# NeLy-EPFL/flygym

Hardware: AMD Instinct MI355X
Metric: env-steps/sec (whole node), 4096 flies per GPU, flat terrain (higher is better)
Workload: dtype f32

## Files before the change

flygym_amd/_native.py:

```python

from __future__ import annotations

import ctypes
import os
import subprocess
from pathlib import Path

PKG = Path(__file__).resolve().parent
LIB_PATH = Path(os.environ["NMF_HIP_LIB"]) if os.environ.get("NMF_HIP_LIB") else PKG / "libnmf_hip.so"
MATH_FLAGS = ["-fno-hip-fp32-correctly-rounded-divide-sqrt", "-freciprocal-math", "-fno-signed-zeros", "-fassociative-math", "-fno-trapping-math", "-fno-math-errno", "-fapprox-func"]
CSRC = PKG / "csrc"
INCLUDE = PKG.parent / "include"

FIELDS = dict(
    qpos=0, qvel=1, ctrl=2, qacc_warmstart=3, seg_xpos=4, seg_xquat=5, site_xpos=6,
    actuator_force=7, sensordata=8, time=9, stats=10, qacc=11, cost=12, stats_sum=13, contact_geom=14, act=15,
)

INT_FIELDS = frozenset({"stats_sum"})

_lib = None


class NativeError(RuntimeError):
    pass


class BatchOptions(ctypes.Structure):

    _fields_ = [("struct_size", ctypes.c_int32), ("solver", ctypes.c_int32), ("sched", ctypes.c_int32), ("order", ctypes.c_int32),
                ("max_chunks", ctypes.c_int32), ("min_chunk_steps", ctypes.c_int32), ("order_every", ctypes.c_int32),
                ("rest_slow", ctypes.c_int32), ("chunk_div", ctypes.c_float), ("flies_per_cu", ctypes.c_int32)]

    SOLVER = {"": 0, "default": 0, "primal": 1, "nohist": 2, "nofallback": 4}
    SCHED = {"": 0, "chunks": 0, "plain": 1}
    ORDER = {"": 0, "auto": 0, "inorder": 1, "costliest": 2, "none": 3, "policy": 4}

    @classmethod
    def make(cls, solver="", sched="", order="", max_chunks=0, min_chunk_steps=0, order_every=0, rest_slow=False, chunk_div=0.0,
             flies_per_cu=0):
        return cls(ctypes.sizeof(cls), cls.SOLVER[solver], cls.SCHED[sched], cls.ORDER[order], int(max_chunks), int(min_chunk_steps),
                   int(order_every), int(bool(rest_slow)), float(chunk_div), int(flies_per_cu))


INFO_KEYS = ("kernel_family", "terrain_kernel", "tether_kernel", "contact_space_flavour", "contact_space_max_contacts", "flies_per_cu",
             "resident_workgroups", "chunked", "max_chunks", "chunk_div_x1000", "order_policy", "solver_option_bits", "noslip_iterations",
             "contact_capacity", "kernel_lds_bytes", "kernel_vgprs")


def build(force: bool = False, verbose: bool = False) -> Path:
    srcs = [CSRC / "nmf_capi.hip", CSRC / "nmf_step.hip", CSRC / "nmf_sensors.hip", CSRC / "nmf_eyes.hip", CSRC / "nmf_replay.hip", CSRC / "nmf_device.h", CSRC / "nmf_tree.h", CSRC / "nmf_dual.h",
            INCLUDE / "nmf.h", Path(__file__)]
    if os.environ.get("NMF_HIP_LIB"):
        return LIB_PATH
    def fresh():
        return LIB_PATH.exists() and all(LIB_PATH.stat().st_mtime >= s.stat().st_mtime for s in srcs)

    if not force and fresh():
        return LIB_PATH
    import fcntl

    lock = open(LIB_PATH.with_suffix(".lock"), "w")
    fcntl.flock(lock, fcntl.LOCK_EX)
    try:
        if not force and fresh():
            return LIB_PATH
        return _compile(verbose)
    finally:
        fcntl.flock(lock, fcntl.LOCK_UN)
        lock.close()


def _compile(verbose: bool) -> Path:
    tmp = LIB_PATH.with_name(LIB_PATH.name + f".{os.getpid()}.tmp")
    cmd = [
        "hipcc", "--offload-arch=gfx950", "-O3", "-std=c++17", "-fno-slp-vectorize", "-mllvm", "-amdgpu-sched-strategy=iterative-ilp",
        *MATH_FLAGS, "-mllvm", "-amdgpu-atomic-optimizer-strategy=None", "-fPIC", "-shared",
        f"-I{INCLUDE}", f"-I{CSRC}", str(CSRC / "nmf_capi.hip"), "-o", str(tmp),
    ]
    res = subprocess.run(cmd, capture_output=True, text=True)
    if res.returncode != 0:
        tmp.unlink(missing_ok=True)
        raise NativeError("hipcc failed:\n" + res.stderr[-4000:])
    if verbose:
        print(res.stderr)
    os.replace(tmp, LIB_PATH)
    return LIB_PATH
# ... 71 lines not shown
```

flygym_amd/csrc/nmf_capi.hip:

```cpp
#include <hip/hip_runtime.h>

#include <algorithm>
#include <cmath>
#include <cstdio>
#include <cstdlib>
#include <cstring>
#include <string>
#include <vector>

#include "nmf.h"
#include "nmf_step.hip"
#include "nmf_sensors.hip"
#include "nmf_eyes.hip"
#include "nmf_replay.hip"

namespace {

thread_local std::string g_err;
int fail(const std::string& msg) { g_err = msg; return -1; }

#define HIP_OK(expr)                                                                        \
  do {                                                                                      \
    hipError_t e_ = (expr);                                                                 \
    if (e_ != hipSuccess) return fail(std::string(#expr) + ": " + hipGetErrorString(e_));   \
// ... 268 lines not shown
  int n_chunks = 1;
  b->st.n_chunks = 1; b->st.csched = b->csched_buf; b->st.handoff = b->handoff_buf; b->st.handoff_stride = b->handoff_stride;
  if (oversub && b->chunking && b->csched_buf && b->handoff_buf && n_steps >= 2 * b->min_chunk_steps) {
    int start = 0, c = 0;
    while (start < n_steps && c < b->max_chunks) {
      const double div = !b->chunk_div_short ? b->chunk_div : n_steps > 64 ? 2.0 : (b->chunk_div < 1.75 && n_steps <= 30 ? 1.6 : b->chunk_div);
      int len = (int)std::ceil((n_steps - start) / div);
      len = std::max(len, b->min_chunk_steps);
      if (c == b->max_chunks - 1 || n_steps - start - len < b->min_chunk_steps) len = n_steps - start;
      b->st.chunk_start[c++] = start;
      start += len;
    }
    b->st.chunk_start[c] = n_steps;
    n_chunks = c;
    b->st.n_chunks = c;
  }
  b->st.sched_mode = n_chunks > 1 ? 1 : 0;
  dim3 grid(n_chunks > 1 ? (unsigned)std::min(b->resident_waves, b->n_worlds * n_chunks) : (unsigned)b->n_worlds), block(nmf::kWave);
  b->st.order = nullptr; b->st.sched = nullptr;
  if (oversub && b->order_buf && b->sched_buf && b->order_policy != 2) {
    const int policy = b->order_policy == 3 ? (n_steps <= 64 ? 1 : -1) : b->order_policy;
    if (!(policy == 1 && b->order_valid && ++b->order_age < b->order_every)) {
      hipLaunchKernelGGL(nmf::nmf_order_kernel, dim3(1), dim3(1024), 0, stream, b->st.cost, b->n_worlds, b->order_buf, b->sched_buf, n_steps, policy);
      b->order_age = 0; b->order_valid = true;
    }
    b->st.order = b->order_buf;
    if (policy < 0) b->st.sched = b->sched_buf;
  }
  const nmf::DevModel* dm = b->dm_dev;
  nmf::ReplayArgs rp_arg = rp;
  void* args[] = {&dm, &b->st, &rp_arg, &n_steps};
  (void)hipLaunchKernel(b->step_fn, grid, block, args, b->lds_pad, stream);
  HIP_OK(hipGetLastError());
  return 0;
}

const char* dev_env(const char* name) {
  static const bool allowed = [] { const char* e = getenv("NMF_ALLOW_ENV"); return e && atoi(e) != 0; }();
  return allowed ? getenv(name) : nullptr;
}

struct Options {
  int solver = 0, sched = 0, order = 0, max_chunks = 0, min_chunk_steps = 0, order_every = 0, rest_slow = 0, flies_per_cu = 0;
  double chunk_div = 0.0;
};

Options read_options(const nmf_batch_options& in) {
  Options o;
  o.solver = in.solver; o.sched = in.sched; o.order = in.order; o.max_chunks = in.max_chunks; o.min_chunk_steps = in.min_chunk_steps;
  o.order_every = in.order_every; o.rest_slow = in.rest_slow; o.flies_per_cu = in.flies_per_cu;
  if (in.chunk_div > 1.f) o.chunk_div = in.chunk_div;
  if (const char* e = dev_env("NMF_SOLVER")) {
    const std::string v(e);
    o.solver = v == "primal" ? 1 : v == "nohist" ? 2 : v == "nofallback" ? 4 : 0;
  }
  if (const char* e = dev_env("NMF_SCHED")) o.sched = std::string(e) == "plain" ? 1 : 0;
  if (const char* e = dev_env("NMF_ORDER")) {
    const std::string v(e);
    o.order = v == "inorder" ? 1 : v == "costliest" ? 2 : v == "none" ? 3 : v == "policy" ? 4 : 0;
  }
  if (const char* e = dev_env("NMF_ORDER_EVERY")) o.order_every = std::max(1, atoi(e));
  if (const char* e = dev_env("NMF_MAX_CHUNKS")) o.max_chunks = std::max(1, std::min(16, atoi(e)));
  if (const char* e = dev_env("NMF_CHUNK_DIV")) o.chunk_div = std::max(1.0, atof(e));
  if (const char* e = dev_env("NMF_MIN_CHUNK_STEPS")) o.min_chunk_steps = std::max(1, atoi(e));
  if (const char* e = dev_env("NMF_FLIES_PER_CU")) o.flies_per_cu = atoi(e);
  if (dev_env("NMF_DISABLE_REST_FAST")) o.rest_slow = 1;
  return o;
}

struct Skeleton {
  int topo = -1;
  std::vector<int> tree_body, child_start, child_count, lvl_start;
};

int classify_skeleton(const nmf_model* model, Skeleton& sk) {
  int& topo = sk.topo;
  if (model->star[0] == 1 && model->star[1] == 6 && model->star[2] == 11 && model->star[3] == 8) topo = 0;
  if (model->star[0] == 1 && model->star[1] == 6 && model->star[2] == 7 && model->star[3] == 4) topo = 1;
  if (topo >= 0) {
    const HostArray* dn = model->find("body_dofnum");
    const int pat0[8] = {3, 2, 1, 1, 1, 1, 1, 1}, pat1[4] = {3, 2, 1, 1};
    const int* pat = topo == 0 ? pat0 : pat1;
    const int nbl = topo == 0 ? 8 : 4;
    bool ok = dn && dn->is_int && (int)dn->i.size() == 1 + 6 * nbl && dn->i[0] == 6;
    for (int b = 1; ok && b < 1 + 6 * nbl; ++b) ok = dn->i[(size_t)b] == pat[(b - 1) % nbl];
    if (!ok || model->nu > nmf::kMaxCtrl) topo = -1;
  }
  std::vector<char> in_tree;
  if (topo < 0) {
    const HostArray* bp = model->find("body_parent");
    const HostArray* dn = model->find("body_dofnum");
    const int patB[8] = {3, 2, 1, 1, 1, 1, 1, 1}, patA[8] = {3, 3, 3, 3, 3, 3, 3, 3};
    for (int cand = 4; cand <= 5 && topo < 0 && bp && dn; ++cand) {
      const int* pat = cand == 4 ? patB : patA;
      const int nb = model->nb, lb0 = 21, want_nv = cand == 4 ? 132 : 210;
      bool ok = nb == 69 && model->nv == want_nv && (int)dn->i.size() == nb && dn->i[0] == 6 && model->nu <= (cand == 4 ? nmf::FlyTopoBio::kCtrl : nmf::FlyTopoAll::kCtrl);
      int rest_v = 0;
      for (int bb = 1; ok && bb < lb0; ++bb) { rest_v += dn->i[(size_t)bb]; ok = bp->i[(size_t)bb] >= 0 && bp->i[(size_t)bb] < lb0 && bp->i[(size_t)bb] < bb; }
      ok = ok && rest_v == 60;
      for (int bb = lb0; ok && bb < nb; ++bb) {
        const int l = (bb - lb0) % 8;
        ok = dn->i[(size_t)bb] == pat[l] && bp->i[(size_t)bb] == (l == 0 ? 0 : bb - 1);
      }
      if (ok) { topo = cand; in_tree.assign((size_t)nb, 0); for (int bb = 0; bb < lb0; ++bb) in_tree[(size_t)bb] = 1; }
    }
  }
  std::vector<int> &tree_body = sk.tree_body, &child_start = sk.child_start, &child_count = sk.child_count, &lvl_start = sk.lvl_start;
// ... 67 lines not shown
  UI(body_dofadr); UI(body_dofnum); UI(dof_body);
  UF(dof_axis); UF(dof_armature); UF(dof_damping); UF(dof_stiffness); UF(dof_springref);
  UI(seg_body); UF(seg_pos); UF(seg_quat); UI(site_body); UF(site_pos);
  UI(act_type); UI(act_trn); UI(act_limited); UI(act_geom); UF(act_gain); UF(act_bias); UF(act_forcerange); UF(act_ctrlrange);
  UF(key_qpos); UF(key_ctrl);
  d.act_general = nullptr;
  if (const HostArray* ag = model->find("act_general")) {
    if (ag->is_int || (int)ag->f.size() != model->nu * nmf::kActGen) { rc |= fail("nmf_batch_create: act_general must be float [nu][32]"); }
    else {
      UF(act_general);
      std::vector<int> trn = model->find("act_trn")->i;
      for (int u = 0; u < model->nu; ++u) if ((int)ag->f[(size_t)u * nmf::kActGen] & 1) trn[(size_t)u] = 0;
      rc |= upload(b, trn, reinterpret_cast<const int**>((void*)&d.act_trn));
    }
  }
  UI(geom_body); UI(geom_type); UI(geom_hulladr); UI(geom_hullnum); UI(geom_sensor);
  UF(geom_p0); UF(geom_p1); UF(geom_radius); UF(geom_bsphere); UF(geom_invweight0); UF(hull_vert);
  UF(pair_friction); UF(pair_solref); UF(pair_solimp); UF(pair_margin);
#undef UF
#undef UI
  if (topo >= 2) {
    const HostArray* bp = model->find("body_parent");
    rc |= upload(b, bp->i, reinterpret_cast<const int**>((void*)&d.body_parent));
    rc |= upload(b, tree_body, reinterpret_cast<const int**>((void*)&d.tree_body));
    rc |= upload(b, child_start, reinterpret_cast<const int**>((void*)&d.tree_child_start));
    rc |= upload(b, child_count, reinterpret_cast<const int**>((void*)&d.tree_child_count));
    d.tree_nlevel = (int)lvl_start.size() - 1;
    for (size_t k = 0; k < 18; ++k) d.tree_lvl_start[k] = k < lvl_start.size() ? lvl_start[k] : (int)tree_body.size();
    d.rest_fast = 0; d.rest_pack = nullptr;
    if (topo >= 4) {
      const HostArray* dn = model->find("body_dofnum");
      const HostArray* da = model->find("body_dofadr");
      const int nl = (int)lvl_start.size() - 2;
      bool fast = da && nl <= nmf::kRestLevels && !opt.rest_slow;
      std::vector<int> pack((size_t)nmf::kRestLevels * 16, -1);
      for (int lv = 1; fast && lv <= nl; ++lv) {
        const int k0 = lvl_start[(size_t)lv], k1 = lvl_start[(size_t)lv + 1];
        fast = k1 - k0 <= 8;
        for (int k = k0; fast && k < k1; ++k) {
          const int bb = tree_body[(size_t)k];
          fast = dn->i[(size_t)bb] == 3 && da->i[(size_t)bb] < 256 && child_count[(size_t)bb] < 256 && child_start[(size_t)bb] < 256;
          pack[(size_t)((lv - 1) * 8 + (k - k0)) * 2] = bb | (bp->i[(size_t)bb] << 8) | (da->i[(size_t)bb] << 16) | (child_count[(size_t)bb] << 24);
          pack[(size_t)((lv - 1) * 8 + (k - k0)) * 2 + 1] = child_start[(size_t)bb] | (k << 8);
        }
      }
      if (fast) { d.rest_fast = 1; const int* pp = nullptr; rc |= upload(b, pack, &pp); *reinterpret_cast<const int**>((void*)&d.rest_pack) = pp; }
    }
  } else {
    d.body_parent = d.tree_body = d.tree_child_start = d.tree_child_count = nullptr; d.tree_nlevel = 0; d.rest_fast = 0; d.rest_pack = nullptr;
  }
  d.noslip_iter = 0;
  if (const HostArray* os2 = model->find("opt_solver")) { if (os2->i.size() > 1) d.noslip_iter = os2->i[1]; }
  d.max_contacts = nmf::kMaxCon;
  d.solver_flags = opt.solver & 7;
  if (rc != 0) return rc;
  void* p = nullptr;
  if (hipMalloc(&p, sizeof(nmf::DevModel)) != hipSuccess) return fail("nmf_batch_create: model upload failed");
  b->allocs.push_back(p); b->dm_dev = (nmf::DevModel*)p;
  if (hipMemcpy(p, &d, sizeof(nmf::DevModel), hipMemcpyHostToDevice) != hipSuccess) return fail("nmf_batch_create: model upload failed");
  return 0;
}

int alloc_state(nmf_batch* b) {
  const nmf_model* model = b->model;
  const size_t n_worlds = (size_t)b->n_worlds;
  nmf::DevState& st = b->st;
  st.n_worlds = b->n_worlds;
  float* stats_sum = nullptr;
  b->handoff_stride = (model->nq + 2 * model->nv + model->nu + 6 + nmf::kActHistWords + 63) / 64 * 64;
  if (alloc_field(b, NMF_QPOS, model->nq, &st.qpos) || alloc_field(b, NMF_QVEL, model->nv, &st.qvel) ||
      alloc_field(b, NMF_CTRL, model->nu, &st.ctrl) || alloc_field(b, NMF_QACC_WARMSTART, model->nv, &st.qacc_ws) ||
      alloc_field(b, NMF_SEG_XPOS, model->nseg * 3, &st.seg_xpos) || alloc_field(b, NMF_SEG_XQUAT, model->nseg * 4, &st.seg_xquat) ||
      alloc_field(b, NMF_SITE_XPOS, model->nsite * 3, &st.site_xpos) || alloc_field(b, NMF_ACTUATOR_FORCE, model->nu, &st.actuator_force) ||
      alloc_field(b, NMF_SENSORDATA, 96, &st.sensordata) || alloc_field(b, NMF_TIME, 1, &st.time) ||
      alloc_field(b, NMF_STATS, 8, &st.stats) || alloc_field(b, NMF_QACC, model->nv, &st.qacc) || alloc_field(b, NMF_COST, 1, &st.cost) ||
      alloc_field(b, NMF_STATS_SUM, 16, &stats_sum) ||
      alloc_field(b, NMF_CONTACT_GEOM, nmf::kMaxCon, &st.contact_geom) || alloc_field(b, NMF_ACT, model->nu, &st.act) ||
      alloc_dev(b, n_worlds, &b->order_buf, false) || alloc_dev(b, 1, &b->csched_buf) ||
      alloc_dev(b, n_worlds * (size_t)b->handoff_stride, &b->handoff_buf) ||
      alloc_dev(b, n_worlds * nmf::kActHistWords, &st.act_hist))
    return -1;
  st.stats_sum = reinterpret_cast<unsigned int*>(stats_sum);
  st.dual_scratch = nullptr;
  if (b->topo == 5 && alloc_dev(b, n_worlds * nmf::kDualScratchFloats, &st.dual_scratch, false)) return -1;
  st.noslip_buf = nullptr;
  if (b->dm.noslip_iter > 0 && alloc_dev(b, n_worlds * nmf::kNoslipFloats, &st.noslip_buf)) return -1;
  if (alloc_dev(b, 2, &b->clock_probe_buf) || alloc_dev(b, 1, &b->sched_buf)) return -1;
  st.clock_probe = b->clock_probe_buf;
  st.sched = nullptr;
  st.order = nullptr;
  return 0;
}

void set_schedule(nmf_batch* b, const Options& opt) {
  b->chunking = opt.sched != 1;
  if (opt.order) b->order_policy = opt.order == 1 ? 0 : opt.order == 2 ? 1 : opt.order == 3 ? 2 : opt.order == 4 ? -1 : 3;
  if (opt.order_every > 0) b->order_every = opt.order_every;
  if (opt.max_chunks > 0) b->max_chunks = std::max(1, std::min(16, opt.max_chunks));
  b->chunk_div = (b->dm.terrain_type == 0 && b->topo < 2) ? 1.7 : 2.0;
  b->chunk_div_short = true;
  if (opt.chunk_div > 0.0) { b->chunk_div = opt.chunk_div; b->chunk_div_short = false; }
  if (opt.min_chunk_steps > 0) b->min_chunk_steps = opt.min_chunk_steps;
  if (b->dm.act_general) b->chunking = false;
}

int pick_kernel(nmf_batch* b, const Options& opt) {
  const int topo = b->topo, device = b->device;
// ... 564 lines not shown
```

flygym_amd/csrc/nmf_dual.h:

```cpp
#pragma once

namespace nmf {

template <class TP>
__device__ __forceinline__ float* dual_g(FlyLds<TP>& s) {
  constexpr size_t need = sizeof(float) * dual_g_floats(kDualMaxCon<TP>);
  if constexpr (kDualH<TP>) {
    static_assert(!kDualH<TP> || need <= sizeof(s.T) + sizeof(s.W), "G does not fit T..W");
    return &s.T[0][0];
  } else {
    static_assert(kDualH<TP> || need <= sizeof(s.Ib) + sizeof(s.T) + sizeof(s.W) + sizeof(s.dual_pad), "G does not fit Ib..W");
    return &s.Ib[0][0];
  }
}
struct DualCol {
  lds_cptr G;
  int cc;
  int cc9b, blk9b;
  int tdb, td3b;
  float smu;
  float alpha, beta;
  struct Raw { float nn, nt, tn, tt, smu2, a2; };
  __device__ __forceinline__ void init(const float* g, int lane, float smu_) {
    G = lds_pinned(g); cc = lane >> 2; cc9b = 36 * cc; blk9b = 36 * (cc * (cc + 1) / 2);
    const int td = 1 + ((lane >> 1) & 1);
    tdb = 4 * td; td3b = 12 * td; smu = smu_;
    alpha = 1.f; beta = smu_;
    asm("" : "+v"(cc9b), "+v"(blk9b), "+v"(tdb), "+v"(td3b));
  }
  __device__ __forceinline__ Raw fetch(int kk) const {
    const unsigned int c2 = (unsigned int)kk >> 2, td2b = 4u + (((unsigned int)kk << 1) & 4u);
    int c29b = (int)(36u * c2), blk29b = (int)(18u * (c2 * (c2 + 1u)));
    asm("" : "+s"(c29b), "+s"(blk29b));
    int lo = blk9b + c29b, up = cc9b + blk29b;
    asm("" : "+v"(lo), "+v"(up));
    const bool ge = cc >= (int)c2;
    const int base = ge ? lo : up;
    const int o_nt = (ge ? 1 : 3) * (int)td2b, o_tn = ge ? td3b : tdb;
    const int a_nt = base + o_nt, a_tn = base + o_tn, a_tt = a_tn + o_nt;
    auto at = [&](int byte_off) { return *(lds_cptr)((const __attribute__((address_space(3))) char*)G + byte_off); };
    Raw r;
    r.nn = at(base); r.nt = at(a_nt); r.tn = at(a_tn); r.tt = at(a_tt);
    r.smu2 = readlane_f(beta, kk); r.a2 = readlane_f(alpha, kk);
    return r;
  }
  __device__ __forceinline__ float value(const Raw& r) const { return fmaf(beta, fmaf(r.smu2, r.tt, r.a2 * r.tn), alpha * fmaf(r.smu2, r.nt, r.a2 * r.nn)); }
};
__device__ __forceinline__ float quad_sum(float v) {
  v += NMF_DPP(v, 0xB1);
  v += NMF_DPP(v, 0x4E);
  return v;
}
constexpr int dual_root_axis(int i) { return i < 3 ? 2 - i : 8 - i; }

template <int PMAX>
__device__ __forceinline__ void dual_eliminate(unsigned long long rem, const DualCol& dc, float R, int lane, float& b, float& diag) {
  float cq[PMAX];
  auto first_of = [](unsigned long long r) { return __builtin_amdgcn_readfirstlane(max(__ffsll((long long)r) - 1, 0)); };
  int kk_next = first_of(rem);
  DualCol::Raw an = dc.fetch(kk_next);
#define NMF_DUAL_PIVOT(P)                                                                                   \
  if constexpr (P < PMAX) {                                                                                 \
    if (rem == 0ull) return;                                                                                \
    const int kk = kk_next;                                                                                 \
    rem &= rem - 1ull;                                                                                      \
    float col = dc.value(an) + (lane == kk ? R : 0.f);                                                      \
    kk_next = first_of(rem);                                                                                \
    an = dc.fetch(kk_next);                                                                                 \
    __builtin_amdgcn_sched_barrier(0);       \
    { float c1 = 0.f;                                                                                       \
      _Pragma("unroll") for (int q = 0; q + 1 < P; q += 2) {                                                \
        col = fmaf(-cq[q], readlane_f(cq[q], kk), col); c1 = fmaf(-cq[q + 1], readlane_f(cq[q + 1], kk), c1); } \
      if constexpr ((P) % 2) col = fmaf(-cq[P - 1], readlane_f(cq[P - 1], kk), col);                        \
      col += c1; }                                                                                          \
    const float d = readlane_f(col, kk);                                                                    \
    const float rs = __builtin_amdgcn_rsqf(d);                                                              \
    diag = lane == kk ? d : diag;                                                                           \
    const float cp = lane == kk ? 0.f : col * rs;                                                           \
    b = fmaf(-cp, readlane_f(b, kk) * rs, b);                                                               \
    cq[P] = cp;                                                                                             \
  }
#define NMF_DUAL_PIVOT8(P) NMF_DUAL_PIVOT(P) NMF_DUAL_PIVOT(P + 1) NMF_DUAL_PIVOT(P + 2) NMF_DUAL_PIVOT(P + 3) NMF_DUAL_PIVOT(P + 4) NMF_DUAL_PIVOT(P + 5) NMF_DUAL_PIVOT(P + 6) NMF_DUAL_PIVOT(P + 7)
  NMF_DUAL_PIVOT8(0) NMF_DUAL_PIVOT8(8) NMF_DUAL_PIVOT8(16) NMF_DUAL_PIVOT8(24) NMF_DUAL_PIVOT8(32) NMF_DUAL_PIVOT8(40) NMF_DUAL_PIVOT8(48) NMF_DUAL_PIVOT8(56)
#undef NMF_DUAL_PIVOT8
#undef NMF_DUAL_PIVOT
}

template <class TP>
__device__ __noinline__ void dual_restore(FlyLds<TP>& s, const GModel& m, int lane) {
  WSYNC();
  if constexpr (kDualS<TP>) {
    for (int b = lane; b < TP::NB; b += kWave) {
      const float* Q = s.Isym[b];
      float* I = s.Ib[b];
      I[0] = Q[15]; I[1] = Q[13]; I[2] = Q[5]; I[3] = Q[8]; I[4] = Q[0]; I[5] = Q[6]; I[6] = Q[11]; I[7] = Q[1]; I[8] = Q[2]; I[9] = Q[7];
    }
    WSYNC();
  }
  sweep_twists(s, s.qacc_smooth, s.T, m, lane);
}

template <class TP>
__device__ __forceinline__ float dual_noslip(FlyLds<TP>& s, const GModel& m, int lane, int ncon, float frow, float j0, float R, float smu) {
  lane = opaque(lane);
  ncon = __builtin_amdgcn_readfirstlane(ncon);
  const bool on = lane < 4 * ncon;
  const float scale = 1.0f / (m.meaninertia * (float)TP::NV);
  DualCol dcol;
  dcol.init(dual_g(s), lane, smu);
    for (int sweep = 0; sweep < m.noslip_iter; ++sweep) {
      float improvement = sweep == 0 ? wave_sum(0.5f * frow * frow * R) : 0.f;
      for (int c2 = 0; c2 < ncon; ++c2) {
        for (int pp = 0; pp < 2; ++pp) {
          const int r0 = 4 * c2 + 2 * pp, r1 = r0 + 1;
          const float col0 = dcol.value(dcol.fetch(r0)), col1 = dcol.value(dcol.fetch(r1));
          const float res0 = wave_sum(on ? col0 * frow : 0.f) + readlane_f(j0, r0), res1 = wave_sum(on ? col1 * frow : 0.f) + readlane_f(j0, r1);
          const float a00 = readlane_f(col0, r0), a01 = readlane_f(col0, r1), a11 = readlane_f(col1, r1);
          const float old0 = readlane_f(frow, r0), old1 = readlane_f(frow, r1);
          const float bc0 = res0 - a00 * old0 - a01 * old1, bc1 = res1 - a01 * old0 - a11 * old1;
          const float mid = 0.5f * (old0 + old1);
          const float K1 = a00 + a11 - 2.f * a01, K0 = mid * (a00 - a11) + bc0 - bc1;
          float n0 = mid, n1 = mid;
          if (!(K1 < kMinVal)) { const float y = fminf(fmaxf(-K0 / K1, -mid), mid); n0 = mid + y; n1 = mid - y; }
          const float d0 = n0 - old0, d1 = n1 - old1;
          float change = 0.5f * (d0 * (a00 * d0 + a01 * d1) + d1 * (a01 * d0 + a11 * d1)) + d0 * res0 + d1 * res1;
          if (change > 1e-10f) { n0 = old0; n1 = old1; change = 0.f; }
          frow = lane == r0 ? n0 : lane == r1 ? n1 : frow;
          improvement -= change;
        }
      }
      if (scale * improvement < 1e-6f) break;
    }
  return frow;
}
template <class TP>
__device__ __noinline__ float dual_noslip_cold(FlyLds<TP>& s, const GModel& m, int lane, int ncon, float frow, float j0, float R, float smu) {
// ... 123 lines not shown
  SUB(43);
  {
    const int kd = k < 3 ? k : 2;
    const int half = ncon >> 1;
    for (int t = 0; t <= half; ++t) {
      int c2 = cc - t;
      c2 = c2 < 0 ? c2 + ncon : c2;
      const int src = (on ? 4 * c2 + k : lane) << 2;
      auto from = [&](float v) { return __builtin_bit_cast(float, __builtin_amdgcn_ds_bpermute(src, __builtin_bit_cast(int, v))); };
      float pr[6], pl[NDL];
#pragma unroll
      for (int i = 0; i < 6; ++i) pr[i] = from(ur[i]);
#pragma unroll
      for (int d = 0; d < NDL; ++d) pl[d] = from(ul[d]);
      const bool same = __builtin_amdgcn_ds_bpermute(src, leg) == leg;
      const bool ge = cc >= c2;
      int base = ge ? 9 * (cc * (cc + 1) / 2 + c2) + 3 * kd : 9 * (c2 * (c2 + 1) / 2 + cc) + kd;
      const int stride = ge ? 1 : 3;
      asm("" : "+v"(base));
      static_for<3>([&](auto PP) {
        constexpr int p = decltype(PP)::value;
        auto rot = [&](float v) {
          if constexpr (p == 0) return v; else if constexpr (p == 1) return NMF_DPP(v, 0xC9); else return NMF_DPP(v, 0xD2);
        };
        float a = rot(pr[0]) * ur[0];
#pragma unroll
        for (int i = 1; i < 6; ++i) a = fmaf(rot(pr[i]), ur[i], a);
        float bl = rot(pl[0]) * ul[0];
#pragma unroll
        for (int d = 1; d < NDL; ++d) bl = fmaf(rot(pl[d]), ul[d], bl);
        a += same ? bl : 0.f;
        const int d2 = kd + p >= 3 ? kd + p - 3 : kd + p;
        if (on && k < 3) Gm[base + stride * d2] = a;
      });
    }
  }
  WSYNC();
  SUB(44);
  STAGE(9);

  float jar = fmaf(c_ws, je, j0), lam = 0.f;
  DualCol dcol;
  dcol.init(Gm, lane, smu);
  const float scale = 1.0f / (m.meaninertia * (float)TP::NV);
  int iters = 0;
  bool guessed = hist_any && !(m.solver_flags & 2);
  int stalls = 0;
  unsigned int exit_bit = kExitMaxIter;
  int npiv = 0;
  float jar_last = 0.f;
  unsigned long long viol_last = 0ull;
  unsigned long long mask_p = ~0ull, mask_pp = ~0ull;
  unsigned long long mask = guessed ? __ballot(on && (hist_nib ? ((hist_nib >> k) & 1) != 0 : jar < 0.f)) : __ballot(on && jar < 0.f);
  for (int iter = 0; iter < m.max_iter; ++iter) {
    iters = iter + 1;
    const unsigned int nib4 = (unsigned int)(mask >> (4 * cc)) & 0xfu;
#ifdef NMF_DUAL_DIRS
    const bool fullc = on && nib4 == 0xfu && mu > 1e-6f;
#else
    const bool fullc = false;
#endif
    float b, diag = 1.f, R_e = R;
    unsigned long long mask_e = mask;
    {
      const float q0 = NMF_DPP(j0, 0x00), q1 = NMF_DPP(j0, 0x55), q2 = NMF_DPP(j0, 0xAA), q3 = NMF_DPP(j0, 0xFF);
      const float hm = 0.5f * __builtin_amdgcn_rcpf(mu);
      const float bdir = k == 0 ? 0.25f * ((q0 + q1) + (q2 + q3)) : k == 1 ? hm * (q0 - q1) : k == 2 ? hm * (q2 - q3) : 0.f;
      b = fullc ? bdir : j0;
      R_e = fullc ? (k == 0 ? 0.25f * R : R * (2.f * hm * hm)) : R;
      dcol.alpha = fullc ? (k == 0 ? 1.f : 0.f) : 1.f;
      dcol.beta = fullc ? ((k == 1 || k == 2) ? 1.f : 0.f) : smu;
      mask_e = __ballot(fullc ? k < 3 : (bool)((mask >> lane) & 1ull));
    }
    dual_eliminate<4 * NC>(mask_e, dcol, R_e, lane, b, diag);
    const bool act = (mask >> lane) & 1ull;
    const bool piv = (mask_e >> lane) & 1ull;
    const float x = piv ? -b * __builtin_amdgcn_rcpf(diag) : 0.f;
    float lam_t, jar_t;
    {
      const float x0 = NMF_DPP(x, 0x00), x1 = NMF_DPP(x, 0x55), x2 = NMF_DPP(x, 0xAA);
      const float hm = 0.5f * __builtin_amdgcn_rcpf(mu);
      const float lam_dir = fmaf((k & 1) ? -hm : hm, k < 2 ? x1 : x2, 0.25f * x0);
      lam_t = fullc ? lam_dir : (act ? x : 0.f);
      jar_t = fullc ? -R * lam_dir : (act ? -R * lam_t : b);
    }
    dcol.alpha = 1.f; dcol.beta = smu;
    const unsigned long long tmask = __ballot(on && jar_t < 0.f);
    npiv = max(npiv, (int)__popcll(mask_e));
    jar_last = jar_t; viol_last = tmask ^ mask;
#ifdef NMF_DUAL_DEBUG
    {
      const float dmin = wave_min(act ? diag : 1e30f), lmax = wave_max(on ? fabsf(lam_t) : 0.f), jmax = wave_max(on ? fabsf(jar_t) : 0.f);
      const float amax = wave_max(on ? fabsf(dcol.value(dcol.fetch(0))) : 0.f);
      if (blockIdx.x == 0 && lane == 0) printf("iter %d npiv %d mask %016llx tmask %016llx min pivot %g max|lam_t| %g max|jar_t| %g max diag A %g c %g\n", iter, __popcll(mask), mask, tmask, dmin, lmax, jmax, amax, c_ws);
    }
#endif
    STAGE(10);
    if (tmask == mask) {
      lam = lam_t; jar = jar_t; c_ws = 0.f;
      exit_bit = kExitKkt;
      break;
    }
    if (iter >= 2 && mask == mask_pp) {
      const bool off = on && (((tmask ^ mask) >> lane) & 1ull);
      const float viol = wave_max(off ? fabsf(jar_t) : 0.f), all = wave_max(on ? fabsf(jar_t) : 0.f);
      if (viol <= 1e-3f * all) { lam = lam_t; jar = jar_t; c_ws = 0.f; exit_bit = kExitTie; break; }
    }
    mask_pp = mask_p; mask_p = mask;
    const float jv = jar_t - jar, dlam = lam_t - lam, dc = -c_ws;
    float g1, g2, s1, s2;
    {
      const float Alam = jar - j0 - c_ws * je, Adlam = fmaf(c_ws, je, jv);
      const bool neg = on && jar < 0.f;
      const float S1 = wave_sum(on ? je * lam : 0.f), S2 = wave_sum(on ? je * dlam : 0.f);
      const float S3 = wave_sum(on ? dlam * Alam : 0.f), S4 = wave_sum(on ? dlam * Adlam : 0.f);
      s1 = wave_sum(neg ? D * jar * jv : 0.f); s2 = wave_sum(neg ? D * jv * jv : 0.f);
      g1 = c_ws * dc * eMe + dc * S1 + c_ws * S2 + S3;
      g2 = dc * dc * eMe + 2.f * dc * S2 + S4;
    }
    STAGE(11);
    float alpha = 0.f, lo = 0.f, hi = -1.f;
    for (int ls = 0; ls < 30; ++ls) {
      float d1 = s1 + g1, d2 = s2 + g2;
      if (ls > 0) {
        const float x = fmaf(alpha, jv, jar);
        const bool neg = on && x < 0.f;
        d1 = wave_sum(neg ? D * x * jv : 0.f) + g1 + alpha * g2;
// ... 173 lines not shown
```

flygym_amd/csrc/nmf_step.hip:

```cpp
#include "nmf_device.h"

namespace nmf {

#define WSYNC() do { __builtin_amdgcn_fence(__ATOMIC_SEQ_CST, "wavefront"); __builtin_amdgcn_wave_barrier(); } while (0)
#ifndef NMF_TOPO_MASK
#define NMF_TOPO_MASK 0x3f
#endif
#define NMF_HAS_TOPO(k) ((NMF_TOPO_MASK >> (k)) & 1)
constexpr float kNoiseFactor = 8.f;
enum : unsigned int {
  kExitDual = 1u << 8,
  kExitKkt = 1u << 9,
  kExitTie = 1u << 10,
  kExitStall = 1u << 11,
  kExitCost = 1u << 12,
  kExitMaxIter = 1u << 13,
  kExitPrimal = 1u << 14,
  kExitFallback = 1u << 15,
  kExitBigPivots = 1u << 16,
  kExitNoNoslip = 1u << 17,
  kExitFree = 1u << 18,
};
constexpr int kExitKinds = 12;
constexpr int kDualRegPivots = 47;
// ... 59 lines not shown
  float fact[TP::kNFact][8];
  float slot[TP::kNSlot][27];
  int rt_nb, rt_nv;
  NMF_TREE_TABLES
};
template <class TP>
struct TreeLds<TP, true, true> {
  float fact[TP::kNFact][8];
  int reduced;
  float restA[21];
  unsigned int t_pack[kRestLevels][8][2];
  NMF_TREE_TABLES
};

template <class TP> constexpr bool has_cm3() { if constexpr (TP::kStar) return TP::REST_B == 0; else return false; }
template <class TP> inline constexpr bool kHasCm3 = has_cm3<TP>();
template <class TP> inline constexpr bool kHasIsym = has_cm3<TP>();

constexpr bool rows_conflict_free(int rows_per_leg, int width, int nleg) {
  const int ng = nleg < 4 ? nleg : 4;
  for (int a = 0; a < ng; ++a)
    for (int b = a + 1; b < ng; ++b) {
      const int d = (((b - a) * rows_per_leg * width) % 32 + 32) % 32;
      if (d < 6 || d > 26) return false;
    }
  return true;
}
constexpr int conflict_free_width(int rows_per_leg, int nleg) {
  for (int w = 6; w <= 9; ++w) if (rows_conflict_free(rows_per_leg, w, nleg)) return w;
  return 6;
}
template <class TP> constexpr int row_width_s() { if constexpr (TP::kStar) return TP::REST_B == 0 ? conflict_free_width(TP::NDL, TP::NLEG) : 6; else return 6; }
template <class TP> constexpr int row_width_tw() { if constexpr (TP::kStar) return TP::REST_B == 0 ? conflict_free_width(TP::NBL, TP::NLEG) : 6; else return 6; }
template <class TP> constexpr bool dual_hybrid() {
  if constexpr (TP::kStar) return TP::REST_B > 0; else return false;
}
template <class TP> constexpr bool dual_global() {
  if constexpr (TP::kStar) return TP::REST_B > 0 && 4 * TP::NV < TP::NLEG * TP::NDL * 8; else return false;
}
template <class TP> inline constexpr bool kDualS = has_cm3<TP>();
template <class TP> inline constexpr bool kDualH = dual_hybrid<TP>();
template <class TP> inline constexpr bool kDual = kDualS<TP> || kDualH<TP>;
template <class TP> inline constexpr bool kDualGlob = kDualH<TP> && dual_global<TP>();
constexpr int kDualScratchFloats = 8 * 6 * 24;
constexpr int dual_g_floats(int ncon) { return 9 * ncon * (ncon + 1) / 2; }
template <class TP> constexpr int dual_max_con() {
  if constexpr (kDualH<TP>) {
    int n = 0;
    while (n < 16 && dual_g_floats(n + 1) <= 2 * TP::NB * 6) ++n;
    return n;
  } else return 16;
}
template <class TP> inline constexpr int kDualMaxCon = dual_max_con<TP>();
template <class TP> inline constexpr int kHistLds = kDualS<TP> ? kActHistWords : kDualH<TP> ? 5 : 0;
template <class TP, class M> __device__ __forceinline__ int hist_words(const M& m) {
  if constexpr (kDualS<TP>) return (m.ng + 1) / 2; else return kHistLds<TP>;
}
template <class TP> constexpr int dual_pad_floats() {
  if constexpr (kDualS<TP>) {
    constexpr int need = dual_g_floats(kDualMaxCon<TP>);
    constexpr int have = TP::NB * 11 + 2 * TP::NB * (TP::REST_B == 0 ? conflict_free_width(TP::NBL, TP::NLEG) : 6);
    return need > have ? need - have : 0;
  } else return 0;
}

struct HotModel {
  const float *dof_axis, *body_pos, *body_quat, *geom_p0, *geom_p1, *geom_radius, *geom_bsphere, *hull_vert, *pair_margin;
  const int *geom_body, *geom_type, *geom_hulladr, *geom_hullnum;
  float plane[4], terrain[5], hull_skin;
  int terrain_type, ng, sem_max_hull_contacts, terrain_walls;
};
template <class TP> struct FlyLds;
template <class TP> struct AbaHandoff;
template <class T> using gptr = const __attribute__((address_space(1))) T*;
template <class T> __device__ __forceinline__ gptr<T> G(const T* p) { return (gptr<T>)p; }
__device__ __forceinline__ V3 ld3(gptr<float> p) { return V3{p[0], p[1], p[2]}; }
__device__ __forceinline__ Q4 ldq(gptr<float> p) { return Q4{p[0], p[1], p[2], p[3]}; }

template <class TP>
struct __align__(16) FlyLds : TreeLds<TP> {
  __device__ __forceinline__ int nv() const { if constexpr (TP::kStar) return TP::NV; else return this->rt_nv; }
  __device__ __forceinline__ int nb() const { if constexpr (TP::kStar) return TP::NB; else return this->rt_nb; }
  __device__ __forceinline__ int nq() const { return nv() + 1; }
  float qpos[TP::NQ + 3];
  float qvel[TP::NV], qacc[TP::NV];
  float xmat_root[9];
  float qacc_smooth[TP::NV], qfrc_smooth[TP::NV];
  float vA[TP::NV], vB[TP::NV], vC[TP::NV], vD[TP::NV];
  float ctrl[TP::kCtrl];
  float S[TP::NV][row_width_s<TP>()];
  float Isym[kHasIsym<TP> ? TP::NB : 1][kHasIsym<TP> ? 21 : 1];
  alignas(kDualS<TP> ? 16 : 4) float Ib[TP::NB][kHasCm3<TP> ? 11 : 10];
  static_assert(6 * TP::NV >= 9 * (TP::NB - 1), "rotation matrices do not fit the solver vectors");
  static_assert(7 * kMaxCon >= 3 * (TP::NB - 1), "body positions do not fit the contact wrenches");
  __device__ __forceinline__ float (*xmat())[9] { return reinterpret_cast<float(*)[9]>(&xmat_root[0]); }
  __device__ __forceinline__ const float (*xmat() const)[9] { return reinterpret_cast<const float(*)[9]>(&xmat_root[0]); }
  __device__ __forceinline__ float (*xpos())[3] { return reinterpret_cast<float(*)[3]>(&xpos_root[0]); }
  __device__ __forceinline__ const float (*xpos() const)[3] { return reinterpret_cast<const float(*)[3]>(&xpos_root[0]); }
  float T[TP::NB][row_width_tw<TP>()], W[TP::NB][row_width_tw<TP>()];
  float dual_pad[dual_pad_floats<TP>()];
  float arm[TP::NV], damp[kHasCm3<TP> ? TP::NV : 1];
  float dlt[kHasCm3<TP> ? TP::NV : 1];
  float c_r[kMaxCon][3], c_D[kMaxCon], c_mu[kMaxCon];
  int c_info[kMaxCon];
  alignas(kDualS<TP> ? 16 : 4) float xpos_pad_[kDualS<TP> ? 1 : 0];
  float xpos_root[3];
// ... 2562 lines not shown
```

Measured before the change: 60.89 million.

## Resume dual active-set factorization from the unchanged pivot prefix between iterations

The dual active-set solver now keeps the Cholesky elimination coefficients (cq) and the forward-solve values (ycol) across iterations. When the new active mask shares a leading prefix with the previously factored one, it replays only the right-hand-side updates for that prefix and jumps into the pivot loop at the first changed pivot. If the mask is unchanged it skips elimination entirely. This adds register pressure from the persistent cq array and a switch-based entry into the unrolled pivot chain. A new solver flag, 'noresume', turns the behaviour off.

New measurement: 56.36 million, median of 2. -7.4%, worse.

```diff
diff --git a/flygym_amd/_native.py b/flygym_amd/_native.py
--- a/flygym_amd/_native.py
+++ b/flygym_amd/_native.py
@@ -32,7 +32,7 @@
                 ("max_chunks", ctypes.c_int32), ("min_chunk_steps", ctypes.c_int32), ("order_every", ctypes.c_int32),
                 ("rest_slow", ctypes.c_int32), ("chunk_div", ctypes.c_float), ("flies_per_cu", ctypes.c_int32)]
 
-    SOLVER = {"": 0, "default": 0, "primal": 1, "nohist": 2, "nofallback": 4}
+    SOLVER = {"": 0, "default": 0, "primal": 1, "nohist": 2, "nofallback": 4, "noresume": 8}
     SCHED = {"": 0, "chunks": 0, "plain": 1}
     ORDER = {"": 0, "auto": 0, "inorder": 1, "costliest": 2, "none": 3, "policy": 4}
 
diff --git a/flygym_amd/csrc/nmf_capi.hip b/flygym_amd/csrc/nmf_capi.hip
--- a/flygym_amd/csrc/nmf_capi.hip
+++ b/flygym_amd/csrc/nmf_capi.hip
@@ -344,7 +344,7 @@
   if (in.chunk_div > 1.f) o.chunk_div = in.chunk_div;
   if (const char* e = dev_env("NMF_SOLVER")) {
     const std::string v(e);
-    o.solver = v == "primal" ? 1 : v == "nohist" ? 2 : v == "nofallback" ? 4 : 0;
+    o.solver = v == "primal" ? 1 : v == "nohist" ? 2 : v == "nofallback" ? 4 : v == "noresume" ? 8 : 0;
   }
   if (const char* e = dev_env("NMF_SCHED")) o.sched = std::string(e) == "plain" ? 1 : 0;
   if (const char* e = dev_env("NMF_ORDER")) {
@@ -518,7 +518,7 @@
   d.noslip_iter = 0;
   if (const HostArray* os2 = model->find("opt_solver")) { if (os2->i.size() > 1) d.noslip_iter = os2->i[1]; }
   d.max_contacts = nmf::kMaxCon;
-  d.solver_flags = opt.solver & 7;
+  d.solver_flags = opt.solver & 15;
   if (rc != 0) return rc;
   void* p = nullptr;
   if (hipMalloc(&p, sizeof(nmf::DevModel)) != hipSuccess) return fail("nmf_batch_create: model upload failed");
diff --git a/flygym_amd/csrc/nmf_dual.h b/flygym_amd/csrc/nmf_dual.h
--- a/flygym_amd/csrc/nmf_dual.h
+++ b/flygym_amd/csrc/nmf_dual.h
@@ -53,13 +53,27 @@
 }
 constexpr int dual_root_axis(int i) { return i < 3 ? 2 - i : 8 - i; }
 
-template <int PMAX>
-__device__ __forceinline__ void dual_eliminate(unsigned long long rem, const DualCol& dc, float R, int lane, float& b, float& diag) {
-  float cq[PMAX];
+template <int PMAX, int K>
+__device__ __forceinline__ void dual_eliminate(unsigned long long rem, unsigned long long pre, int m, const DualCol& dc, float R, int lane,
+                                               float& b, float& diag, float (&cq)[PMAX], float& ycol) {
+  static_assert(K >= 0 && K < PMAX, "the resumable prefix is a part of the pivot blocks");
   auto first_of = [](unsigned long long r) { return __builtin_amdgcn_readfirstlane(max(__ffsll((long long)r) - 1, 0)); };
   int kk_next = first_of(rem);
   DualCol::Raw an = dc.fetch(kk_next);
+  if constexpr (K > 0) {
+#define NMF_DUAL_REPLAY(Q)                                                                                  \
+    if constexpr (Q < K) {                                                                                  \
+      if (pre == 0ull) goto replayed;                                                                       \
+      { const int kq = first_of(pre); pre &= pre - 1ull; b = fmaf(-cq[Q], readlane_f(ycol, kq), b); }       \
+    }
+#define NMF_DUAL_REPLAY8(Q) NMF_DUAL_REPLAY(Q) NMF_DUAL_REPLAY(Q + 1) NMF_DUAL_REPLAY(Q + 2) NMF_DUAL_REPLAY(Q + 3) NMF_DUAL_REPLAY(Q + 4) NMF_DUAL_REPLAY(Q + 5) NMF_DUAL_REPLAY(Q + 6) NMF_DUAL_REPLAY(Q + 7)
+    NMF_DUAL_REPLAY8(0) NMF_DUAL_REPLAY8(8) NMF_DUAL_REPLAY8(16) NMF_DUAL_REPLAY8(24) NMF_DUAL_REPLAY8(32) NMF_DUAL_REPLAY8(40) NMF_DUAL_REPLAY8(48) NMF_DUAL_REPLAY8(56)
+#undef NMF_DUAL_REPLAY8
+#undef NMF_DUAL_REPLAY
+  }
+replayed:
 #define NMF_DUAL_PIVOT(P)                                                                                   \
+  case ((P) <= K ? (P) : -1 - (P)):                                                                         \
   if constexpr (P < PMAX) {                                                                                 \
     if (rem == 0ull) return;                                                                                \
     const int kk = kk_next;                                                                                 \
@@ -77,11 +91,16 @@
     const float rs = __builtin_amdgcn_rsqf(d);                                                              \
     diag = lane == kk ? d : diag;                                                                           \
     const float cp = lane == kk ? 0.f : col * rs;                                                           \
-    b = fmaf(-cp, readlane_f(b, kk) * rs, b);                                                               \
+    const float y = readlane_f(b, kk) * rs;                                                                 \
+    if constexpr (P < K) ycol = lane == kk ? y : ycol;                                                      \
+    b = fmaf(-cp, y, b);                                                                                    \
     cq[P] = cp;                                                                                             \
   }
 #define NMF_DUAL_PIVOT8(P) NMF_DUAL_PIVOT(P) NMF_DUAL_PIVOT(P + 1) NMF_DUAL_PIVOT(P + 2) NMF_DUAL_PIVOT(P + 3) NMF_DUAL_PIVOT(P + 4) NMF_DUAL_PIVOT(P + 5) NMF_DUAL_PIVOT(P + 6) NMF_DUAL_PIVOT(P + 7)
+  switch (K > 0 ? m : 0) {
+  default:
   NMF_DUAL_PIVOT8(0) NMF_DUAL_PIVOT8(8) NMF_DUAL_PIVOT8(16) NMF_DUAL_PIVOT8(24) NMF_DUAL_PIVOT8(32) NMF_DUAL_PIVOT8(40) NMF_DUAL_PIVOT8(48) NMF_DUAL_PIVOT8(56)
+  }
 #undef NMF_DUAL_PIVOT8
 #undef NMF_DUAL_PIVOT
 }
@@ -311,6 +330,15 @@
   unsigned long long viol_last = 0ull;
   unsigned long long mask_p = ~0ull, mask_pp = ~0ull;
   unsigned long long mask = guessed ? __ballot(on && (hist_nib ? ((hist_nib >> k) & 1) != 0 : jar < 0.f)) : __ballot(on && jar < 0.f);
+  constexpr int KR = kDualResume<TP>;
+  float cq[4 * NC];
+  float b = 0.f, diag = 1.f, ycol = 0.f;
+  unsigned long long mask_done = 0ull;
+  bool kept = false;
+  const bool resume = KR > 0 && !(m.solver_flags & 8);
+#ifdef NMF_DUAL_DIRS
+  unsigned long long full_done = 0ull;
+#endif
   for (int iter = 0; iter < m.max_iter; ++iter) {
     iters = iter + 1;
     const unsigned int nib4 = (unsigned int)(mask >> (4 * cc)) & 0xfu;
@@ -319,19 +347,43 @@
 #else
     const bool fullc = false;
 #endif
-    float b, diag = 1.f, R_e = R;
+    float b0, R_e = R;
     unsigned long long mask_e = mask;
     {
       const float q0 = NMF_DPP(j0, 0x00), q1 = NMF_DPP(j0, 0x55), q2 = NMF_DPP(j0, 0xAA), q3 = NMF_DPP(j0, 0xFF);
       const float hm = 0.5f * __builtin_amdgcn_rcpf(mu);
       const float bdir = k == 0 ? 0.25f * ((q0 + q1) + (q2 + q3)) : k == 1 ? hm * (q0 - q1) : k == 2 ? hm * (q2 - q3) : 0.f;
-      b = fullc ? bdir : j0;
+      b0 = fullc ? bdir : j0;
       R_e = fullc ? (k == 0 ? 0.25f * R : R * (2.f * hm * hm)) : R;
       dcol.alpha = fullc ? (k == 0 ? 1.f : 0.f) : 1.f;
       dcol.beta = fullc ? ((k == 1 || k == 2) ? 1.f : 0.f) : smu;
       mask_e = __ballot(fullc ? k < 3 : (bool)((mask >> lane) & 1ull));
     }
-    dual_eliminate<4 * NC>(mask_e, dcol, R_e, lane, b, diag);
+    {
+      bool same_sys = kept;
+#ifdef NMF_DUAL_DIRS
+      const unsigned long long full_e = __ballot(fullc);
+      same_sys = same_sys && full_e == full_done;
+      full_done = full_e;
+#endif
+      const unsigned long long diff = mask_e ^ mask_done;
+      unsigned long long pre = mask_e & ((diff & (0ull - diff)) - 1ull);
+      int mpre = __popcll(pre);
+#ifdef NMF_STAGE_PROFILE
+      {
+        const int P = __popcll(mask_e), ms = !same_sys ? 0 : diff == 0ull ? P : mpre <= KR ? mpre : 0;
+        SUB_COUNT(35, 1); SUB_COUNT(41, same_sys && diff == 0ull ? 1 : 0); SUB_COUNT(42, P); SUB_COUNT(45, iter > 0 ? P : 0);
+        SUB_COUNT(46, ms); SUB_COUNT(47, 52 * ms + ms * (ms - 1));
+      }
+#endif
+      if (!(resume && same_sys)) { pre = 0ull; mpre = 0; }
+      if (!(resume && same_sys && diff == 0ull)) {
+        if (mpre > KR) { pre = 0ull; mpre = 0; }
+        b = b0;
+        dual_eliminate<4 * NC, KR>(mask_e ^ pre, pre, mpre, dcol, R_e, lane, b, diag, cq, ycol);
+      }
+      mask_done = mask_e; kept = true;
+    }
     const bool act = (mask >> lane) & 1ull;
     const bool piv = (mask_e >> lane) & 1ull;
     const float x = piv ? -b * __builtin_amdgcn_rcpf(diag) : 0.f;
diff --git a/flygym_amd/csrc/nmf_step.hip b/flygym_amd/csrc/nmf_step.hip
--- a/flygym_amd/csrc/nmf_step.hip
+++ b/flygym_amd/csrc/nmf_step.hip
@@ -135,6 +135,7 @@
   } else return 16;
 }
 template <class TP> inline constexpr int kDualMaxCon = dual_max_con<TP>();
+template <class TP> inline constexpr int kDualResume = kDualH<TP> ? 0 : TP::kTerrain ? 16 : kDualRegPivots;
 template <class TP> inline constexpr int kHistLds = kDualS<TP> ? kActHistWords : kDualH<TP> ? 5 : 0;
 template <class TP, class M> __device__ __forceinline__ int hist_words(const M& m) {
   if constexpr (kDualS<TP>) return (m.ng + 1) / 2; else return kHistLds<TP>;
```
